# izhengfan/se2lam

Hardware: AMD Instinct MI355X
Metric: BA GN-iters/s (200 KF, 20k pts) (higher is better)
Workload: dtype f64; 1 GPU; globalBA-window 200 KF / 20000 landmarks / 119817 EdgeSE2XYZ + 199 PreEdgeSE2, LM optimize(10) (config 4 formulation, SURVEY D3); parallelism=single GPU

## Files before the change

### se2lam_amd/csrc/ba.hip

```cpp
#include <algorithm>
#include <atomic>
#include <chrono>
#include <cmath>
#include <cstdlib>
#include <functional>
#include <limits>
#include <mutex>
#include <thread>
#include <memory>
#include <unordered_map>

#include "common.h"
#include "se3_math.h"
#include "ba_device.h"
#include "ba3_device.h"
#include "ba_window.h"

using namespace se2gpu;
using namespace se2gpu::badev;

namespace {



// ... 2 lines not shown
    for (int r = 0; r < 3; ++r) {
        const double h0 = hh[r * 3], h1 = hh[r * 3 + 1], h2 = hh[r * 3 + 2];
        w[r * 3 + 0] = h0 * a[0];
        w[r * 3 + 1] = h0 * a[1] + h1 * a[2];
        w[r * 3 + 2] = h0 * a[3] + h1 * a[4] + h2 * a[5];
    }
}
__device__ __forceinline__ void edge_record(const double* __restrict__ hh, const double* __restrict__ hp,
                                            const double* __restrict__ bpe, const double a[6], const double zeta[3],
                                            double w[9], double dg[12]) {
    edge_w(hh, a, w);
    dg[0] = hp[0] - (w[0] * w[0] + w[1] * w[1] + w[2] * w[2]);
    dg[1] = hp[1] - (w[0] * w[3] + w[1] * w[4] + w[2] * w[5]);
    dg[2] = hp[2] - (w[0] * w[6] + w[1] * w[7] + w[2] * w[8]);
    dg[3] = hp[3] - (w[3] * w[3] + w[4] * w[4] + w[5] * w[5]);
    dg[4] = hp[4] - (w[3] * w[6] + w[4] * w[7] + w[5] * w[8]);
    dg[5] = hp[5] - (w[6] * w[6] + w[7] * w[7] + w[8] * w[8]);
#pragma unroll
    for (int r = 0; r < 3; ++r) {
        dg[6 + r] = bpe[r];
        dg[9 + r] = w[r * 3] * zeta[0] + w[r * 3 + 1] * zeta[1] + w[r * 3 + 2] * zeta[2];
    }
}
__device__ inline void write_edge_record(double* __restrict__ w_out, double* __restrict__ dg_out, const double* __restrict__ hh,
                                         const double* __restrict__ hp, const double* __restrict__ bpe,
                                         const double a[6], const double zeta[3]) {
    double w[9], dg[12];
    edge_record(hh, hp, bpe, a, zeta, w, dg);
#pragma unroll
    for (int i = 0; i < 9; ++i) w_out[i] = w[i];
#pragma unroll
    for (int i = 0; i < 12; ++i) dg_out[i] = dg[i];
}

__device__ __forceinline__ void wave_copy_out(double* __restrict__ dst, const double* stage, int n) {
    const int lane = threadIdx.x & 63;
    const int head = (int)((reinterpret_cast<uintptr_t>(dst) >> 3) & 1);
    if (lane == 0 && head) dst[0] = stage[0];
    const int nb = (n - head) >> 1;
    for (int i = lane; i < nb; i += 64) {
        const double2 v = make_double2(stage[head + 2 * i], stage[head + 2 * i + 1]);
        *reinterpret_cast<double2*>(dst + head + 2 * i) = v;
    }
    if (lane == 0 && ((n - head) & 1)) dst[n - 1] = stage[n - 1];
}

struct RecSet {
    double *W, *Dg, *Hll, *bl, *Ainv, *zeta;
};

__device__ __forceinline__ void lin_edge(const CamDev& cam, double px, double py, double pth, double lx, double ly, double lz,
                                         double u, double v, double w0, double w1, double w2, bool fr, double hll[6],
                                         double b[3], double hpl[9], double hpp[6], double bpe[3], double& r0) {
    double e0, e1, Jp[6], Jl[6];
    se2xyz<true>(cam, px, py, pth, lx, ly, lz, u, v, e0, e1, Jp, Jl);
// ... 42 lines not shown
        double* keep = lds + (threadIdx.x >> 6) * kWaveLds + (threadIdx.x & 63);
#pragma unroll
        for (int i = 0; i < 9; ++i) keep[i * 64] = hpl[i];
#pragma unroll
        for (int i = 0; i < 6; ++i) keep[(9 + i) * 64] = hpp[i];
#pragma unroll
        for (int i = 0; i < 3; ++i) keep[(15 + i) * 64] = bpe[i];
    } else {
        if (FUSED) {
#pragma unroll
            for (int i = 0; i < 9; ++i) W[(size_t)e * 9 + i] = hpl[i];
        }
#pragma unroll
        for (int i = 0; i < 6; ++i) Hpp_e[(size_t)e * 6 + i] = hpp[i];
#pragma unroll
        for (int i = 0; i < 3; ++i) bp_e[(size_t)e * 3 + i] = bpe[i];
    }
}

template <bool FUSED>
__device__ __forceinline__ void lin_landmark(int l, int sub, int beg, int end, int L, double hll[6], double b[3], double lambda,
                                             double* lds, double* W, double* Hpp_e, double* bp_e,
                                             double* __restrict__ Hll, double* __restrict__ bl, double* __restrict__ Ainv,
                                             double* __restrict__ zeta, double* __restrict__ Dg) {
#pragma unroll
    for (int i = 0; i < 6; ++i) hll[i] = group_sum(hll[i]);
#pragma unroll
    for (int i = 0; i < 3; ++i) b[i] = group_sum(b[i]);
    if (l < L && sub == 0) {
#pragma unroll
        for (int i = 0; i < 6; ++i) Hll[(size_t)l * 6 + i] = hll[i];
#pragma unroll
        for (int i = 0; i < 3; ++i) bl[(size_t)l * 3 + i] = b[i];
    }
    if (!FUSED) return;
    int e1 = l < L ? end : 0;
#pragma unroll
    for (int o = 32; o; o >>= 1) e1 = max(e1, __shfl_xor(e1, o));
    const int E0 = __builtin_amdgcn_readfirstlane(l < L ? beg : 0), E1 = __builtin_amdgcn_readfirstlane(e1);
    const int ne = E1 - E0;
    const bool staged = ne > 0 && ne <= kStageEdges;
    double* stage = lds + (threadIdx.x >> 6) * kWaveLds;
    const double* keep = stage + (threadIdx.x & 63);
    const bool has = l < L && beg + sub < end;
    double a[6] = {0, 0, 0, 0, 0, 0}, zt[3] = {0, 0, 0};
    if (l < L) {
        chol_inv3(hll, lambda, a);
        zt[0] = a[0] * b[0];
        zt[1] = a[1] * b[0] + a[2] * b[1];
        zt[2] = a[3] * b[0] + a[4] * b[1] + a[5] * b[2];
        if (sub == 0) {
#pragma unroll
            for (int i = 0; i < 6; ++i) Ainv[(size_t)l * 6 + i] = a[i];
#pragma unroll
            for (int i = 0; i < 3; ++i) zeta[(size_t)l * 3 + i] = zt[i];
        }
    }
    double w1[9], dg1[12];
    if (has) {
        double k_hpl[9], k_hpp[6], k_bp[3];
#pragma unroll
        for (int i = 0; i < 9; ++i) k_hpl[i] = keep[i * 64];
#pragma unroll
        for (int i = 0; i < 6; ++i) k_hpp[i] = keep[(9 + i) * 64];
#pragma unroll
        for (int i = 0; i < 3; ++i) k_bp[i] = keep[(15 + i) * 64];
        edge_record(k_hpl, k_hpp, k_bp, a, zt, w1, dg1);
    }
    const int lend = l < L ? end : 0;
    if (!staged) {
        if (has) {
#pragma unroll
            for (int i = 0; i < 9; ++i) W[(size_t)(beg + sub) * 9 + i] = w1[i];
#pragma unroll
            for (int i = 0; i < 12; ++i) Dg[(size_t)(beg + sub) * 12 + i] = dg1[i];
        }
        for (int e = beg + sub + kGroup; e < lend; e += kGroup) {
            double hh[9], hp[6], bpe[3];
#pragma unroll
            for (int i = 0; i < 9; ++i) hh[i] = W[(size_t)e * 9 + i];
#pragma unroll
            for (int i = 0; i < 6; ++i) hp[i] = Hpp_e[(size_t)e * 6 + i];
#pragma unroll
            for (int i = 0; i < 3; ++i) bpe[i] = bp_e[(size_t)e * 3 + i];
            write_edge_record(W + (size_t)e * 9, Dg + (size_t)e * 12, hh, hp, bpe, a, zt);
        }
        return;
    }
    __builtin_amdgcn_wave_barrier();
    if (has) {
#pragma unroll
        for (int i = 0; i < 12; ++i) stage[(beg + sub - E0) * 12 + i] = dg1[i];
    }
    for (int e = beg + sub + kGroup; e < lend; e += kGroup) {
        double hh[9], hp[6], bpe[3], w[9], dg[12];
#pragma unroll
        for (int i = 0; i < 9; ++i) hh[i] = W[(size_t)e * 9 + i];
#pragma unroll
        for (int i = 0; i < 6; ++i) hp[i] = Hpp_e[(size_t)e * 6 + i];
#pragma unroll
        for (int i = 0; i < 3; ++i) bpe[i] = bp_e[(size_t)e * 3 + i];
        edge_record(hh, hp, bpe, a, zt, w, dg);
#pragma unroll
        for (int i = 0; i < 12; ++i) stage[(e - E0) * 12 + i] = dg[i];
    }
    __builtin_amdgcn_wave_barrier();
    wave_copy_out(Dg + (size_t)E0 * 12, stage, ne * 12);
    __builtin_amdgcn_wave_barrier();
    if (has) {
#pragma unroll
        for (int i = 0; i < 9; ++i) stage[(beg + sub - E0) * 9 + i] = w1[i];
    }
    for (int e = beg + sub + kGroup; e < lend; e += kGroup) {
        double hh[9], w[9];
#pragma unroll
        for (int i = 0; i < 9; ++i) hh[i] = W[(size_t)e * 9 + i];
        edge_w(hh, a, w);
#pragma unroll
        for (int i = 0; i < 9; ++i) stage[(e - E0) * 9 + i] = w[i];
    }
    __builtin_amdgcn_wave_barrier();
    wave_copy_out(W + (size_t)E0 * 9, stage, ne * 9);
}

struct LinArgs {
    CamDev cam;
    int L;
    const int *lm_ptr, *e_kf;
    const double *e_uv, *e_info, *poses;
    const uint8_t* fixed;
    const double* lms;
    double *W, *Hpp_e, *bp_e, *Hll, *bl;
    double lambda;
    double *Ainv, *zeta, *Dg;
    const BaCtl* ctl;
    const double *poses_b, *lms_b;
    RecSet alt;
};
template <bool FUSED>
__device__ __forceinline__ void d_linearize(const unsigned bx, const LinArgs& a) {
    const double *poses = a.poses, *lms = a.lms;
    RecSet rec{a.W, a.Dg, a.Hll, a.bl, a.Ainv, a.zeta};
    double lambda = a.lambda;
    if constexpr (FUSED) asm volatile("" : "+s"(lambda));
    if (a.ctl) {
        if (a.ctl->done | a.ctl->rec_valid) return;
        if (a.ctl->sel) { poses = a.poses_b; lms = a.lms_b; }
        if (a.ctl->rec_sel) rec = a.alt;
        lambda = a.ctl->lambda;
    }
    const int gid = bx * kBlock + threadIdx.x;
    const int l = gid / kGroup, sub = gid % kGroup;
    double hll[6] = {0, 0, 0, 0, 0, 0}, b[3] = {0, 0, 0};
    __shared__ double keep[(kBlock / 64) * kWaveLds];
    int beg = 0, end = 0;
    if (l < a.L) {
        const double lx = lms[3 * l], ly = lms[3 * l + 1], lz = lms[3 * l + 2];
        beg = a.lm_ptr[l];
        end = a.lm_ptr[l + 1];
        for (int e = beg + sub; e < end; e += kGroup) {
            const int kf = a.e_kf[e];
            double hpl[9], hpp[6], bpe[3], r0;
            lin_edge(a.cam, poses[3 * kf], poses[3 * kf + 1], poses[3 * kf + 2], lx, ly, lz, a.e_uv[2 * e], a.e_uv[2 * e + 1],
                     a.e_info[3 * e], a.e_info[3 * e + 1], a.e_info[3 * e + 2], !a.fixed[kf], hll, b, hpl, hpp, bpe, r0);
            lin_park<FUSED>(e == beg + sub, e, hpl, hpp, bpe, keep, rec.W, a.Hpp_e, a.bp_e);
        }
    }
    lin_landmark<FUSED>(l, sub, beg, end, a.L, hll, b, lambda, keep, rec.W, a.Hpp_e, a.bp_e, rec.Hll, rec.bl, rec.Ainv, rec.zeta,
                        rec.Dg);
}
template <bool FUSED>
__global__ __launch_bounds__(kBlock) void k_linearize(LinArgs a) {
    d_linearize<FUSED>(blockIdx.x, a);
}


struct OdoArgs {
    int O;
    const int *o_i, *o_j;
    const double *o_meas, *o_info, *poses;
    const uint8_t* fixed;
    double *Oii, *Ojj, *Oij, *obi, *obj;
    const BaCtl* ctl;
    const double* poses_b;
};
__device__ __forceinline__ void d_odometry(const unsigned bx, const OdoArgs& a) {
    const double* poses = a.poses;
    if (a.ctl && a.ctl->sel) poses = a.poses_b;
    const int k = bx * blockDim.x + threadIdx.x;
    if (k >= a.O) return;
    const int i = a.o_i[k], j = a.o_j[k];
    double e[3], A[9], B[9];
// ... 192 lines not shown
    const int i = o_i[k], j = o_j[k];
    pre_se2(poses + 3 * i, poses + 3 * j, o_meas + 3 * k, e, A, B);
    const double* W = o_info + 9 * k;
    for (int r = 0; r < 3; ++r) {
        omr[r] = -(W[r * 3] * e[0] + W[r * 3 + 1] * e[1] + W[r * 3 + 2] * e[2]);
        for (int c = 0; c < 3; ++c) {
            WA[r * 3 + c] = W[r * 3] * A[c] + W[r * 3 + 1] * A[3 + c] + W[r * 3 + 2] * A[6 + c];
            WB[r * 3 + c] = W[r * 3] * B[c] + W[r * 3 + 1] * B[3 + c] + W[r * 3 + 2] * B[6 + c];
        }
    }
}

constexpr int kGrpPerWG = 28;
constexpr int kChunk = 16;

struct Reduce2Args {
    int P, ld, nwg_off;
    double lambda;
    int root;
    const int4* grp;
    const int *blk_a, *blk_b, *pair_i, *pair_j, *blk_odo;
    const double *W, *Dg;
    const uint8_t* fixed;
    const int *pose_ptr, *pose_edges, *podo_ptr, *podo_item, *o_i, *o_j;
    const double *o_meas, *o_info, *poses;
    double *S, *bp;
    const BaCtl* ctl;
    const double* poses_b;
    unsigned* epoch;
    const int* pose_off;
    int nsys;
    const double *W_alt, *Dg_alt;
};
__device__ __forceinline__ void d_reduce2(const unsigned bx, const Reduce2Args& ra) {
    const double *W = ra.W, *Dg = ra.Dg, *poses = ra.poses;
    if (ra.ctl && ra.ctl->rec_sel) { W = ra.W_alt; Dg = ra.Dg_alt; }
    double lambda = ra.lambda;
    const int n = ra.pose_off ? ra.nsys : 3 * ra.P;
    __shared__ double part[kGrpPerWG][9];
    __shared__ double dpart[kBlock / 64][12];
    const int ndiag = (ra.P + 1 + 7) & ~7;
    if ((int)bx >= ndiag) {
        const int bid = (int)bx - ndiag;
        const int nwg_pad = (ra.nwg_off + 7) & ~7;
        const int wg = (bid & 7) * (nwg_pad >> 3) + (bid >> 3);
        if (wg >= ra.nwg_off) return;
        const int lane = threadIdx.x & 63, gw = lane / 9, en = lane - 9 * gw;
// ... 94 lines not shown
    double acc[12] = {0, 0, 0, 0, 0, 0, 0, 0, 0, 0, 0, 0};
    const bool fa = ra.fixed[p];
    __shared__ double odoc[8][12];
    const int no = fa ? 0 : ra.podo_ptr[p + 1] - ra.podo_ptr[p];
    if ((int)threadIdx.x >= kBlock - 8 && (int)threadIdx.x - (kBlock - 8) < min(no, 8)) {
        const int t = ra.podo_ptr[p] + (int)threadIdx.x - (kBlock - 8);
        const int k = ra.podo_item[t] >> 1, isj = ra.podo_item[t] & 1;
        double e[3], A[9], B[9], WA[9], WB[9], omr[3];
        odo_terms(poses, ra.fixed, ra.o_i, ra.o_j, ra.o_meas, ra.o_info, k, e, A, B, WA, WB, omr);
        double J[9], WJ[9];
#pragma unroll
        for (int t9 = 0; t9 < 9; ++t9) { J[t9] = isj ? B[t9] : A[t9]; WJ[t9] = isj ? WB[t9] : WA[t9]; }
        double* o = odoc[threadIdx.x - (kBlock - 8)];
#pragma unroll
        for (int r = 0; r < 3; ++r) {
#pragma unroll
            for (int c = 0; c < 3; ++c) o[r * 3 + c] = J[r] * WJ[c] + J[3 + r] * WJ[3 + c] + J[6 + r] * WJ[6 + c];
            o[9 + r] = J[r] * omr[0] + J[3 + r] * omr[1] + J[6 + r] * omr[2];
        }
    }
    if (!fa) {
        const int e0 = ra.pose_ptr[p], ne = ra.pose_ptr[p + 1] - e0;
        for (int base = 0; base < ne; base += 4 * kBlock) {
            int ee[4];
            double wgt[4];
#pragma unroll
            for (int u = 0; u < 4; ++u) {
                const int t = base + u * kBlock + (int)threadIdx.x;
                wgt[u] = t < ne ? 1.0 : 0.0;
                ee[u] = ra.pose_edges[e0 + min(t, ne - 1)];
            }
#pragma unroll
            for (int u = 0; u < 4; ++u) {
                if (base + u * kBlock >= ne) break;
                const double2* rec = reinterpret_cast<const double2*>(Dg + (size_t)ee[u] * 12);
                const double w = wgt[u];
#pragma unroll
                for (int i = 0; i < 6; ++i) {
                    const double2 v = rec[i];
                    acc[2 * i] += w * v.x;
                    acc[2 * i + 1] += w * v.y;
                }
            }
        }
    }
#pragma unroll
    for (int i = 0; i < 12; ++i) acc[i] = wave_sum(acc[i]);
    if (lane == 0) {
#pragma unroll
        for (int i = 0; i < 12; ++i) dpart[wv][i] = acc[i];
    }
    __syncthreads();
    if (threadIdx.x < 12) {
        const int i = threadIdx.x;
        const int sym[9] = {0, 1, 2, 1, 3, 4, 2, 4, 5};
        const int src = i < 9 ? sym[i] : i - 3;
        double v = dpart[0][src] + dpart[1][src] + dpart[2][src] + dpart[3][src];
        for (int t = 0; t < min(no, 8); ++t) v += odoc[t][i];
        for (int t = ra.podo_ptr[p] + 8; t < ra.podo_ptr[p] + no; ++t) {
// ... 645 lines not shown
    TrialEnd te;
};
__device__ void finish_trial(const FinArgs& fin, const double* part, double lambda, double* fsp);

struct SpecArgs {
    RecSet set[2];
    double *Hpp_e, *bp_e;
};

struct UpdArgs {
    CamDev cam;
    int L;
    double lambda;
    const int *lm_ptr, *e_kf;
    const double *e_uv, *e_info, *poses;
    const uint8_t* fixed;
    const double *lms, *xp, *zeta, *W, *bl;
    double *lms_trial, *part;
    const BaCtl* ctl;
    const double* poses_b;
    FinArgs fin;
    const double* Ainv;
    SpecArgs sp;
};
template <bool LIN>
__device__ __forceinline__ void d_update(const unsigned bx, const UpdArgs& a) {
    __shared__ double lds[LIN ? (kBlock / 64) * kWaveLds : 3 * 1024];
    static_assert((kBlock / 64) * kWaveLds >= 3 * 1024, "the finisher's pose stage");
    if (a.fin.enabled && (int)bx == a.fin.nblk) {
        finish_trial(a.fin, a.part, a.lambda, lds);
        return;
    }
    const double *poses = a.poses, *lms = a.lms, *zeta = a.zeta, *W = a.W, *bl = a.bl, *Ainv = a.Ainv;
    double* lms_trial = a.lms_trial;
    double lambda = a.lambda;
    const int gid = bx * kBlock + threadIdx.x;
    const int l = gid / kGroup, sub = gid % kGroup;
    int beg = 0, end = 0;
    if (l < a.L) {
        beg = a.lm_ptr[l];
        end = a.lm_ptr[l + 1];
    }
    if (a.ctl) {
        if (a.ctl->done) return;
        if (a.ctl->sel) {
            const double* t = lms; lms = lms_trial; lms_trial = const_cast<double*>(t);
            poses = a.poses_b;
        }
        lambda = a.ctl->lambda;
    }
    const bool step = a.xp != nullptr;
    bool spec = false;
    double lambda_spec = 0;
    RecSet wr{};
    if (LIN && a.ctl && step) {
        spec = a.ctl->it + 1 < a.ctl->iters;
        lambda_spec = lm_lambda_spec(lambda, a.ctl->mode);
        const int rs = a.ctl->rec_sel;
        const RecSet rd = a.sp.set[rs];
        wr = a.sp.set[rs ^ 1];
        W = rd.W; zeta = rd.zeta; bl = rd.bl; Ainv = rd.Ainv;
    }
    double* keep = lds;
    double hll[6] = {0, 0, 0, 0, 0, 0}, bsum[3] = {0, 0, 0};
    __shared__ double sm[2][kBlock / 64];
    double chi = 0, scale = 0;
    double x[3] = {0, 0, 0};
    constexpr int KS = 2;
    int ekf[KS];
    bool ev[KS];
    double ey[KS][9], ep[KS][3], epose[KS][3], euv[KS][2], ew[KS][3];
    bool efix[KS];
#pragma unroll
    for (int k = 0; k < KS; ++k) {
        const int e = beg + sub + k * kGroup;
        ev[k] = e < end;
        const int ec = ev[k] ? e : max(end - 1, 0);
        const bool has = l < a.L && end > beg;
        ekf[k] = has ? a.e_kf[ec] : 0;
#pragma unroll
        for (int i = 0; i < 9; ++i) ey[k][i] = (has && step) ? W[(size_t)ec * 9 + i] : 0.0;
        euv[k][0] = has ? a.e_uv[2 * (size_t)ec] : 0.0;
        euv[k][1] = has ? a.e_uv[2 * (size_t)ec + 1] : 0.0;
#pragma unroll
        for (int i = 0; i < 3; ++i) ew[k][i] = has ? a.e_info[3 * (size_t)ec + i] : 0.0;
    }
#pragma unroll
    for (int k = 0; k < KS; ++k) {
        const int kf = ekf[k];
        epose[k][0] = poses[3 * kf]; epose[k][1] = poses[3 * kf + 1]; epose[k][2] = poses[3 * kf + 2];
        efix[k] = a.fixed[kf] != 0;
#pragma unroll
        for (int i = 0; i < 3; ++i) ep[k][i] = step ? a.xp[3 * kf + i] : 0.0;
    }
    double lw0[3] = {0, 0, 0}, zz[3] = {0, 0, 0}, blv[3] = {0, 0, 0}, av[6] = {0, 0, 0, 0, 0, 0};
    if (l < a.L) {
#pragma unroll
        for (int c = 0; c < 3; ++c) {
            lw0[c] = lms[(size_t)l * 3 + c];
            if (step) { zz[c] = zeta[(size_t)l * 3 + c]; blv[c] = bl[(size_t)l * 3 + c]; }
        }
        if (step) {
// ... 65 lines not shown
            edge_chi(e, poses[3 * kf], poses[3 * kf + 1], poses[3 * kf + 2], a.fixed[kf] != 0, dp, a.e_uv[2 * e], a.e_uv[2 * e + 1],
                     a.e_info[3 * e], a.e_info[3 * e + 1], a.e_info[3 * e + 2]);
        }
    }
    chi = wave_sum(chi);
    scale = wave_sum(scale);
    const int w = threadIdx.x / 64;
    if ((threadIdx.x & 63) == 0) { sm[0][w] = chi; sm[1][w] = scale; }
    __syncthreads();
    if (threadIdx.x == 0) {
        double c = 0, s = 0;
        for (int i = 0; i < kBlock / 64; ++i) { c += sm[0][i]; s += sm[1][i]; }
        if (a.fin.enabled) {
            store_agent(a.part + 2 * bx, d2_t{c, s});
            asm volatile("s_waitcnt vmcnt(0)" ::: "memory");
            __hip_atomic_fetch_add(a.fin.counter, 1u, __ATOMIC_RELAXED, __HIP_MEMORY_SCOPE_AGENT);
        } else {
            a.part[2 * bx] = c;
            a.part[2 * bx + 1] = s;
        }
    }
    if (LIN && spec)
        lin_landmark<true>(l, sub, beg, end, a.L, hll, bsum, lambda_spec, keep, wr.W, a.sp.Hpp_e, a.sp.bp_e, wr.Hll, wr.bl, wr.Ainv,
                           wr.zeta, wr.Dg);
}
template <bool LIN>
__global__ __launch_bounds__(kBlock) void k_update(UpdArgs a) {
    d_update<LIN>(blockIdx.x, a);
}

__global__ void k_ctl_clear_error(BaCtl* __restrict__ ctl) {
    ctl->error = 0;
    ctl->done = 0;
}

__device__ inline void post_ctl(const BaCtl* c, volatile double* mail, double seq, int tid, int nthr) {
    constexpr int kWords = (int)(sizeof(BaCtl) / 8);
    const double* src = reinterpret_cast<const double*>(c);
    for (int i = tid; i < kWords; i += nthr) mail[8 + i] = src[i];
}

__device__ inline void end_slot(BaCtl* ctl, volatile double* mail, bool post, int tid, int nthr, bool step) {
    if (!step) return;
    if (tid == 0) ctl->seq += 1.0;
    __syncthreads();
    if (post && mail) {
        __threadfence();
// ... 1011 lines not shown
    std::vector<int> pg_perm;
    DevBuf<int> slot_a, slot_ptr, pe_i, pe_j;
    DevBuf<double> pe_meas, pe_info, ph;
    int bulk_E = 0;
    const int32_t *bulk_kf = nullptr, *bulk_lm = nullptr;
    const double *bulk_uv = nullptr, *bulk_info = nullptr;
    bool lg_active = false;
    std::vector<float> lg_lc, lg_lw, lg_sigma2, lg_Rcw, lg_twb;
    float lg_fx = 0, lg_srot = 0, lg_sz = 0;
    DevBuf<float> d_lg_lc, d_lg_lw, d_lg_sigma2, d_lg_Rcw, d_lg_twb;
    std::vector<EdgeOdo> odo;
    bool initialized = false;
    unsigned long init_serial = 0;
    hipEvent_t join_event = nullptr;
    hipStream_t join_stream = nullptr;
    bool own_pending = false;
    int P = 0, L = 0, E = 0, O = 0, nblk = 0, nparts = 0;
    int ld = 0;
    bool host_solve = false;
    DevBuf<double> poses0, lms0, poses_a, poses_b, lms_a, lms_b;
    double *poses = nullptr, *poses_t = nullptr, *lms = nullptr, *lms_t = nullptr;
    DevBuf<uint8_t> fixed;
    DevBuf<int> lm_ptr, e_kf, e_lm, pose_ptr, pose_edges, podo_ptr, podo_item, o_i, o_j;
    DevBuf<int> blk_a, blk_b, blk_ptr, pair_i, pair_j, blk_odo;
    DevBuf<int4> grp;
    int nwg_off = 0, grp_cap_wg = 0;
    DevBuf<uint8_t> garena;
    DevBuf<int> plan_np, plan_base, plan_key0, plan_key1, plan_idx, plan_hist, plan_offs, plan_out, plan_tsum, plan_toff;
    DevBuf<int2> plan_st0, plan_st1;
    bool odo_fallback = false;
    bool odo_self_loop = false;
    DevBuf<double> e_uv, e_info, o_meas, o_info;
    DevBuf<double> Hpl, Hpp_e, bp_e, Hll, bl, Dinv, z, Y, Dg, Hpp, bp, Oii, Ojj, Oij, obi, obj;
    DevBuf<double> red_own, xp, part, scal, diag3, Rinv;
    DevBuf<double> rec_twin;
    bool run_spec = false;
    DevBuf<double> red_packed;
    DevBuf<int4> chol_tasks;
    DevBuf<int> chol_deps;
    DevBuf<int> chol_neager;
    DevBuf<int> pose_off;
    DevBuf<int> col_src;
    std::vector<int> h_pose_off;
    DevBuf<uint8_t> plan_nz;
    DevBuf<double> plan_nzd;
    PinBuf<uint8_t> h_plan_nz;
// ... 413 lines not shown
    if ((int)blockIdx.x < b1) {
        const int l = blockIdx.x * 256 + threadIdx.x;
        if (l >= L) return;
        int o = pair_base[l];
        const int beg = lm_ptr[l], end = lm_ptr[l + 1];
        for (int s = beg; s < end; ++s) {
            const int a = e_kf[s];
            if (fixed[a]) continue;
            for (int t = s + 1; t < end; ++t) {
                const int b = e_kf[t];
                if (fixed[b] || a == b) continue;
                const int q = a < b ? blk_index_of(P, a, b) : blk_index_of(P, b, a);
                key[o] = q;
                st[o] = a < b ? make_int2(s, t) : make_int2(t, s);
                if (nz) nz[q] = 1;
                ++o;
            }
        }
    } else {
        const int i = (blockIdx.x - b1) * 256 + threadIdx.x;
        if (i < cap && i >= pair_base[L]) key[i] = big;
    }
}
__global__ __launch_bounds__(256) void k_plan_bounds(const int* __restrict__ key, int n, int nq, int* __restrict__ out,
                                                      const int2* __restrict__ st, int* __restrict__ pi, int* __restrict__ pj,
                                                      int b1) {
    if ((int)blockIdx.x < b1) {
        const int q = blockIdx.x * 256 + threadIdx.x;
        if (q > nq) return;
        int lo = 0, hi = n;
        while (lo < hi) {
            const int mid = (lo + hi) >> 1;
            if (key[mid] < q) lo = mid + 1; else hi = mid;
        }
        out[q] = lo;
    } else {
        const int i = (blockIdx.x - b1) * 256 + threadIdx.x;
        if (i < n) { pi[i] = st[i].x; pj[i] = st[i].y; }
    }
}
inline dim3 grid1(size_t n, int block) { return dim3((unsigned)std::max<size_t>((n + block - 1) / block, 1)); }

__global__ void k_pattern_widen(int n, uint8_t* __restrict__ nz, double* __restrict__ d, int dir) {
    const int i = blockIdx.x * blockDim.x + threadIdx.x;
    if (i >= n) return;
    if (dir == 0) d[i] = nz[i] ? 1.0 : 0.0;
    else nz[i] = d[i] > 0.5 ? 1 : 0;
}
__global__ void k_solver_pads(double* __restrict__ S, int ld, int nsys, const int* __restrict__ col_src) {
    const int c = blockIdx.x * blockDim.x + threadIdx.x;
    if (c < nsys && col_src[c] < 0) S[(size_t)c * ld + c] = 1.0;
}

struct HostPlan {
    std::vector<int> lm_ptr, pose_ptr, pose_edges, blk_a, blk_b, blk_odo, pair_i, pair_j;
    std::vector<uint8_t> blk_nz;
    std::vector<int4> grp;
    int nwg_off = 0;
};
void ba_plan_host(int P, int L, int E, const int* e_kf, const int* e_lm, const uint8_t* fx, int O, const int* o_i,
                  const int* o_j, bool odo_ok, HostPlan& pl, int gpw = kGrpPerWG) {
    pl.lm_ptr.assign(L + 1, 0);
    for (int s = 0; s < E; ++s) pl.lm_ptr[e_lm[s] + 1]++;
    for (int l = 0; l < L; ++l) pl.lm_ptr[l + 1] += pl.lm_ptr[l];
    const std::vector<int>& lm_ptr = pl.lm_ptr;
    pl.pose_ptr.assign(P + 1, 0);
    pl.pose_edges.resize(E);
    for (int s = 0; s < E; ++s) pl.pose_ptr[e_kf[s] + 1]++;
    for (int p = 0; p < P; ++p) pl.pose_ptr[p + 1] += pl.pose_ptr[p];
    {
        std::vector<int> f(pl.pose_ptr.begin(), pl.pose_ptr.end() - 1);
        for (int s = 0; s < E; ++s) pl.pose_edges[f[e_kf[s]]++] = s;
    }
    const int nblk = P * (P + 1) / 2;
    std::vector<int> blk_ptr(nblk + 1, 0);
    pl.blk_a.resize(nblk);
    pl.blk_b.resize(nblk);
    for (int a = 0; a < P; ++a)
        for (int b = a; b < P; ++b) {
            pl.blk_a[blk_index_of(P, a, b)] = a;
            pl.blk_b[blk_index_of(P, a, b)] = b;
        }
    std::vector<int> pkey;
    std::vector<int2> pst;
    pkey.reserve(4 * (size_t)E);
    pst.reserve(4 * (size_t)E);
    for (int l = 0; l < L; ++l)
        for (int s = lm_ptr[l]; s < lm_ptr[l + 1]; ++s) {
            const int a = e_kf[s];
            if (fx[a]) continue;
            for (int t = s + 1; t < lm_ptr[l + 1]; ++t) {
                const int b = e_kf[t];
                if (fx[b] || a == b) continue;
                const int q = a < b ? blk_index_of(P, a, b) : blk_index_of(P, b, a);
                pkey.push_back(q);
                pst.push_back(a < b ? make_int2(s, t) : make_int2(t, s));
// ... 429 lines not shown
        stage(h->pe_j, pg_j.data(), pg_j.size());
        stage(h->pe_meas, pg_meas.data(), pg_meas.size());
        stage(h->pe_info, pg_info.data(), pg_info.size());
    }
    if (h->model) {
        stage(h->prior_has, h->h_prior_has.data(), h->h_prior_has.size());
        stage(h->prior_meas, h->h_prior_meas.data(), h->h_prior_meas.size());
        stage(h->prior_info, h->h_prior_info.data(), h->h_prior_info.size());
    }
    if (h->lg_active) {
        SE2_REQUIRE(sorted && h->lg_sigma2.size() == (size_t)E, SE2GPU_ERR_STATE,
                    "load_local_graph must not be mixed with add_edge calls");
        stage(h->d_lg_lc, h->lg_lc.data(), h->lg_lc.size());
        stage(h->d_lg_lw, h->lg_lw.data(), h->lg_lw.size());
        stage(h->d_lg_sigma2, h->lg_sigma2.data(), h->lg_sigma2.size());
        stage(h->d_lg_Rcw, h->lg_Rcw.data(), h->lg_Rcw.size());
        stage(h->d_lg_twb, h->lg_twb.data(), h->lg_twb.size());
    }
    if (!device_plan) {
        stage(h->grp, pl.grp.data(), pl.grp.size());
        stage(h->lm_ptr, pl.lm_ptr.data(), pl.lm_ptr.size());
        stage(h->pose_ptr, pl.pose_ptr.data(), pl.pose_ptr.size());
        stage(h->pose_edges, pl.pose_edges.data(), pl.pose_edges.size());
        stage(h->blk_a, pl.blk_a.data(), pl.blk_a.size());
        stage(h->blk_b, pl.blk_b.data(), pl.blk_b.size());
        stage(h->blk_odo, pl.blk_odo.data(), pl.blk_odo.size());
        stage(h->pair_i, pl.pair_i.data(), pl.pair_i.size());
        stage(h->pair_j, pl.pair_j.data(), pl.pair_j.size());
    }
    SE2_CHECK(h->poses_a.reserve((size_t)ps * P));
    SE2_CHECK(h->poses_b.reserve((size_t)ps * P));
    SE2_CHECK(h->lms_a.reserve(3 * (size_t)L + 1));
    SE2_CHECK(h->lms_b.reserve(3 * (size_t)L + 1));
    SE2_CHECK(h->Hpl.reserve((size_t)D * 3 * E + 1));
    if (h->model) SE2_CHECK(h->Y.reserve((size_t)D * 3 * E + 1));
    SE2_CHECK(h->Hpp_e.reserve((size_t)DS * E + 1));
    SE2_CHECK(h->bp_e.reserve((size_t)D * E + 1));
    SE2_CHECK(h->Dg.reserve((size_t)(DS + 2 * D) * E + 1));
    SE2_CHECK(h->Hll.reserve(6 * (size_t)L + 1));
    SE2_CHECK(h->bl.reserve(3 * (size_t)L + 1));
    SE2_CHECK(h->Dinv.reserve(6 * (size_t)L + 1));
    SE2_CHECK(h->z.reserve(3 * (size_t)L + 1));
    SE2_CHECK(h->Hpp.reserve((size_t)D * D * P));
    SE2_CHECK(h->bp.reserve((size_t)D * P));
    SE2_CHECK(h->diag3.reserve((size_t)D * P));
    SE2_CHECK(h->Oii.reserve((size_t)D * D * O + 1));
// ... 68 lines not shown
                done += nb;
                if (sg.off + done - sent >= kPiece) SE2_CHECK(flush_on(sg.off + done));
            }
        }
        return flush_on(std::min(hi, staged_bytes));
    };
    for (const Staged& sg : staged) sg.bind(h->garena.p + sg.off);
    SE2_CHECK(stage_range(0, big_off, st));
    lap("indices staged");
    bool pattern_early = false;
    if (h->lg_active && E)
        hipLaunchKernelGGL(k_edge_information, grid1(E, 256), dim3(256), 0, st, E, h->d_lg_lc.p, h->d_lg_lw.p, h->e_kf.p,
                           h->d_lg_sigma2.p, h->d_lg_Rcw.p, h->d_lg_twb.p, h->lg_fx, h->lg_srot, h->lg_sz, h->e_info.p, 1);
    if (device_plan) {
        const int Pb = std::max(1, (int)std::ceil(std::log2((double)std::max(P, 2))));
        const int Qb = std::max(2, (int)std::ceil(std::log2((double)nblk + 2.0)));
        const int qlo = (Qb + 1) / 2, qhi = Qb - qlo;
        SE2_REQUIRE(qlo <= 10 && Pb <= 10, SE2GPU_ERR_CAPACITY, "device plan: %d poses", P);
        const size_t NP = std::max<size_t>(npairs_max, 1);
        const int nblkE = (int)((E + kRadixItems - 1) / kRadixItems), nblkP = (int)((NP + kRadixItems - 1) / kRadixItems);
        SE2_CHECK(h->lm_ptr.reserve((size_t)L + 2));
        SE2_CHECK(h->pose_ptr.reserve((size_t)P + 2));
        SE2_CHECK(h->pose_edges.reserve((size_t)E + 1));
        SE2_CHECK(h->blk_a.reserve(nblk));
        SE2_CHECK(h->blk_b.reserve(nblk));
        SE2_CHECK(h->blk_odo.reserve(nblk));
        SE2_CHECK(h->blk_ptr.reserve((size_t)nblk + 2));
        SE2_CHECK(h->pair_i.reserve(NP));
        SE2_CHECK(h->pair_j.reserve(NP));
        SE2_CHECK(h->plan_np.reserve((size_t)L + 2));
        SE2_CHECK(h->plan_base.reserve((size_t)L + 2));
        SE2_CHECK(h->plan_key0.reserve(std::max<size_t>(NP, (size_t)E + 1)));
        SE2_CHECK(h->plan_key1.reserve(std::max<size_t>(NP, (size_t)E + 1)));
        SE2_CHECK(h->plan_st0.reserve(NP));
        SE2_CHECK(h->plan_st1.reserve(NP));
        SE2_CHECK(h->plan_idx.reserve((size_t)E + 1));
        const size_t nhist = (size_t)1024 * std::max(nblkE, nblkP) + 2;
        SE2_CHECK(h->plan_hist.reserve(nhist));
        SE2_CHECK(h->plan_offs.reserve(nhist));
        SE2_CHECK(h->plan_out.reserve(8));
        SE2_CHECK(h->plan_tsum.reserve(nhist / kScanTile + 4));
        SE2_CHECK(h->plan_toff.reserve(nhist / kScanTile + 4));
        const size_t G = npairs_max / kChunk + (size_t)P * (P - 1) / 2 + 1;
        const int cap_wg = (int)std::min<size_t>((size_t)P * (P - 1) / 2 + 1, 2 * G / gpw + 2) + 1;
        SE2_CHECK(h->grp.reserve((size_t)cap_wg * gpw));
        h->grp_cap_wg = cap_wg;
// ... 15 lines not shown
                               (int)cnt, shift, bins, nb, h->plan_offs.p, kout, vout);
            return SE2GPU_OK;
        };
        uint8_t* nzp = nullptr;
        if (nd_possible) {
            SE2_CHECK(h->plan_nz.reserve((size_t)nblk));
            SE2_CHECK(h->h_plan_nz.reserve((size_t)nblk));
            nzp = h->plan_nz.p;
        }
        {
            const int g1 = (int)grid1((size_t)L + 1, 256).x, g2 = (int)grid1(E, 256).x, g3 = (int)grid1((size_t)P * P, 256).x;
            const size_t ngrp = (size_t)cap_wg * gpw;
            const int g4 = (int)grid1(ngrp, 256).x;
            hipLaunchKernelGGL(k_plan_init, dim3(g1 + g2 + g3 + g4), dim3(256), 0, st, L, E, P, h->e_lm.p, h->e_kf.p, h->fixed.p,
                               h->lm_ptr.p, h->plan_np.p, h->plan_idx.p, h->blk_a.p, h->blk_b.p, h->blk_odo.p, ngrp, h->grp.p,
                               g1, g1 + g2, g1 + g2 + g3, nzp);
        }
        hipLaunchKernelGGL(k_scan_i32, dim3(1), dim3(1024), 0, st, h->plan_np.p, h->plan_base.p, L);
        if (O && (!h->odo_fallback || nzp))
            hipLaunchKernelGGL(k_plan_odo, grid1(O, 64), dim3(64), 0, st, P, O, h->o_i.p, h->o_j.p,
                               h->odo_fallback ? nullptr : h->blk_odo.p, nzp);
        if (E) SE2_CHECK(radix(h->e_kf.p, h->plan_key0.p, h->plan_idx.p, h->pose_edges.p, (size_t)E, 0, Pb));
        hipLaunchKernelGGL(k_lower_bounds, grid1((size_t)P + 1, 256), dim3(256), 0, st, h->plan_key0.p, E, P, h->pose_ptr.p);
        {
            const int g1 = (int)grid1(L, 256).x, g2 = (int)grid1(NP, 256).x;
            hipLaunchKernelGGL(k_plan_pairs2, dim3(g1 + g2), dim3(256), 0, st, L, P, h->lm_ptr.p, h->e_kf.p, h->fixed.p,
                               h->plan_base.p, h->plan_key0.p, h->plan_st0.p, (int)NP, nblk, g1, nzp);
        }
        if (nd_possible) {
            if (nd_sharded) {
                SE2_CHECK(h->plan_nzd.reserve((size_t)nblk));
                hipLaunchKernelGGL(k_pattern_widen, grid1((size_t)nblk, 256), dim3(256), 0, st, nblk, h->plan_nz.p, h->plan_nzd.p, 0);
                SE2_HIP(hipGetLastError());
                SE2_CHECK(ba_allreduce(h, h->plan_nzd.p, (size_t)nblk));
                hipLaunchKernelGGL(k_pattern_widen, grid1((size_t)nblk, 256), dim3(256), 0, st, nblk, h->plan_nz.p, h->plan_nzd.p, 1);
            }
            SE2_HIP(hipMemcpyAsync(h->h_plan_nz.p, h->plan_nz.p, (size_t)nblk, hipMemcpyDeviceToHost, st));
            SE2_HIP(hipEventRecord(h->ev_pat, st));
            pattern_early = true;
        }
        SE2_CHECK(radix(h->plan_key0.p, h->plan_key1.p, h->plan_st0.p, h->plan_st1.p, NP, 0, qlo));
        SE2_CHECK(radix(h->plan_key1.p, h->plan_key0.p, h->plan_st1.p, h->plan_st0.p, NP, qlo, std::max(qhi, 1)));
        {
            const int g1 = (int)grid1((size_t)nblk + 1, 256).x, g2 = (int)grid1(NP, 256).x;
            hipLaunchKernelGGL(k_plan_bounds, dim3(g1 + g2), dim3(256), 0, st, h->plan_key0.p, (int)NP, nblk, h->blk_ptr.p,
                               h->plan_st0.p, h->pair_i.p, h->pair_j.p, g1);
// ... 171 lines not shown
    for (unsigned i = t0; i < it.np; i += stride) it.dst_p[i] = it.src_p[i];
    for (unsigned i = t0; i < it.nl; i += stride) it.dst_l[i] = it.src_l[i];
}

struct Bufs {
    const BaCtl* c;
    double *pa, *pb, *la, *lb;
};
inline Bufs bufs(se2gpu_ba* h, bool ctl) {
    if (ctl) return Bufs{h->ctl.p, h->poses_a.p, h->poses_b.p, h->lms_a.p, h->lms_b.p};
    return Bufs{nullptr, h->poses, h->poses_t, h->lms, h->lms_t};
}

bool ba_env_speculate() {
    static const bool on = env_flag("SE2GPU_BA_SPECULATE", true);
    return on;
}
RecSet rec_own(const se2gpu_ba* h) { return RecSet{h->Hpl.p, h->Dg.p, h->Hll.p, h->bl.p, h->Dinv.p, h->z.p}; }
RecSet rec_twin(const se2gpu_ba* h) {
    if (!h->rec_twin.p || h->model) return RecSet{};
    const size_t E = (size_t)h->E, L = (size_t)h->L;
    double* p = h->rec_twin.p;
    RecSet r;
    r.W = p; p += 9 * E + 1;
    r.Dg = p; p += 12 * E + 1;
    r.Hll = p; p += 6 * L + 1;
    r.bl = p; p += 3 * L + 1;
    r.Ainv = p; p += 6 * L + 1;
    r.zeta = p;
    return r;
}
int ba_reserve_twin(se2gpu_ba* h) { return h->rec_twin.reserve(21 * (size_t)h->E + 18 * (size_t)h->L + 6); }

inline double* ba_scal(se2gpu_ba* h) { return h->red + (size_t)h->ld * h->ld; }
inline dim3 upd_grid(const se2gpu_ba* h) { return grid1((size_t)h->L * kGroup, kBlock); }
inline dim3 reduce2_grid(const se2gpu_ba* h) { return dim3(((h->P + 1 + 7) & ~7) + ((h->nwg_off + 7) & ~7)); }
LinArgs lin_args(se2gpu_ba* h, const Bufs& B, double lambda, const RecSet& alt) {
    return LinArgs{h->cam, h->L, h->lm_ptr.p, h->e_kf.p, h->e_uv.p, h->e_info.p, B.pa, h->fixed.p, B.la, h->Hpl.p, h->Hpp_e.p,
                   h->bp_e.p, h->Hll.p, h->bl.p, lambda, h->Dinv.p, h->z.p, h->Dg.p, B.c, B.pb, B.lb, alt};
}
OdoArgs odo_args(se2gpu_ba* h, const double* poses, bool ctl) {
    const Bufs B = bufs(h, ctl);
    return OdoArgs{h->O, h->o_i.p, h->o_j.p, h->o_meas.p, h->o_info.p, ctl ? B.pa : poses, h->fixed.p, h->Oii.p, h->Ojj.p, h->Oij.p,
                   h->obi.p, h->obj.p, B.c, ctl ? B.pb : nullptr};
}
PoseReduceArgs pose_reduce_args(se2gpu_ba* h) {
    return PoseReduceArgs{h->P, h->pose_ptr.p, h->pose_edges.p, h->Hpp_e.p, h->bp_e.p, h->podo_ptr.p, h->podo_item.p, h->Oii.p,
                          h->Ojj.p, h->obi.p, h->obj.p, h->Hpp.p, h->bp.p};
}
MaxdiagArgs maxdiag_args(se2gpu_ba* h, int dpp, int stride9, BaCtl* ctl) {
    return MaxdiagArgs{h->L, h->Hll.p, h->P, stride9 ? h->Hpp.p : h->diag3.p, h->fixed.p, h->scal.p, dpp, stride9, ctl};
}
Reduce2Args reduce2_args(se2gpu_ba* h, const Bufs& B, double lambda, const RecSet& alt) {
    return Reduce2Args{h->P, h->ld, h->nwg_off, lambda, h->root, h->grp.p, h->blk_a.p, h->blk_b.p, h->pair_i.p, h->pair_j.p,
                       h->blk_odo.p, h->Hpl.p, h->Dg.p, h->fixed.p, h->pose_ptr.p, h->pose_edges.p, h->podo_ptr.p, h->podo_item.p,
                       h->o_i.p, h->o_j.p, h->o_meas.p, h->o_info.p, B.pa, h->red, h->bp.p, B.c, B.pb, &h->ctl.p->epoch,
                       h->pose_off.p, h->nsys, alt.W, alt.Dg};
}
CholArgs chol_args(se2gpu_ba* h, const BaCtl* ctl, int skip, unsigned long long* head, bool verify) {
    const int n = h->nsys, ld = h->ld;
    const int nt = ld / kNB, nbc = (n + kNB - 1) / kNB;
    double* YU = h->Rinv.p + 2 * (size_t)nt * nbc * kSlabs * kSlabDoubles;
    unsigned* flagA = h->chol_flags.p;
    return CholArgs{h->red, h->Rinv.p, YU, ld, n, nbc, h->chol_tasks.p + skip, h->chol_deps.p, h->chol_neager.p + skip, h->col_src.p,
                    flagA, flagA + kSlabs * (size_t)nt * nbc, &h->ctl.p->epoch, ba_scal(h) + 2, h->chol_trace.p, ctl, h->xp.p,
                    verify ? h->chol_vfy.p : nullptr, head, h->chol_ntask - skip};
}
TrialEnd trial_end(se2gpu_ba* h, const Bufs& B, int step, int decide, int notify, double seq, bool lin = false, bool post = true) {
    return TrialEnd{ba_scal(h), post ? h->d_mail : nullptr, seq, B.c ? h->ctl.p : nullptr,
                    B.c ? (const volatile int*)h->d_stop : nullptr, step, decide, notify, lin ? 1 : 0};
}
FinArgs fin_args(se2gpu_ba* h, const Bufs& B, const double* xp, const TrialEnd& te) {
    return FinArgs{1, (int)upd_grid(h).x, h->P, h->O, h->root, h->fixed.p, xp, h->bp.p, B.pa, B.pb,
                   h->o_i.p, h->o_j.p, h->o_meas.p, h->o_info.p, h->fin_counter.p, te};
}
UpdArgs upd_args(se2gpu_ba* h, const Bufs& B, double lambda, const double* xp, const FinArgs& fin, bool lin = false) {
    return UpdArgs{h->cam, h->L, lambda, h->lm_ptr.p, h->e_kf.p, h->e_uv.p, h->e_info.p, B.pa, h->fixed.p, B.la, xp, h->z.p, h->Hpl.p,
                   h->bl.p, B.lb, h->part.p, B.c, B.pb, fin, h->Dinv.p,
                   lin ? SpecArgs{{rec_own(h), rec_twin(h)}, h->Hpp_e.p, h->bp_e.p} : SpecArgs{}};
}


int ba_linearize(se2gpu_ba* h, double fuse_lambda, bool ctl = false) {
    hipStream_t st = h->stream;
    const Bufs B = bufs(h, ctl);
    if (h->model == 2) {
        SE2_LAUNCH(h->prof, st, "k4_terms", k4_terms, grid1((size_t)h->P + h->O, 64), dim3(64), 0, h->P, h->O, B.pa, h->fixed.p,
                   h->prior_has.p, h->prior_meas.p, h->prior_info.p, h->ph.p, h->pb.p, h->slot_a.p, h->slot_ptr.p, h->pe_i.p,
                   h->pe_j.p, h->pe_meas.p, h->pe_info.p, h->Oii.p, h->Ojj.p, h->Oij.p, h->obi.p, h->obj.p, B.c, B.pb);
        SE2_HIP(hipGetLastError());
        return SE2GPU_OK;
    }
    if (h->model) {
        if (fuse_lambda >= 0.0)
            SE2_LAUNCH(h->prof, st, "k3_linearize", (k3_linearize<true>), grid1((size_t)h->L * kGroup, kBlock), dim3(kBlock), 0,
                       h->cam3, h->L, h->lm_ptr.p, h->e_kf.p, h->e_uv.p, h->e_info.p, B.pa, h->fixed.p, B.la, h->Hpl.p,
                       h->Hpp_e.p, h->bp_e.p, h->Hll.p, h->bl.p, fuse_lambda, h->Dinv.p, h->z.p, h->Y.p, h->Dg.p, B.c, B.pb, B.lb);
        else
            SE2_LAUNCH(h->prof, st, "k3_linearize", (k3_linearize<false>), grid1((size_t)h->L * kGroup, kBlock), dim3(kBlock), 0,
                       h->cam3, h->L, h->lm_ptr.p, h->e_kf.p, h->e_uv.p, h->e_info.p, B.pa, h->fixed.p, B.la, h->Hpl.p,
                       h->Hpp_e.p, h->bp_e.p, h->Hll.p, h->bl.p, 0.0, h->Dinv.p, h->z.p, h->Y.p, h->Dg.p, B.c, B.pb, B.lb);
        SE2_LAUNCH(h->prof, st, "k3_terms", k3_terms, grid1((size_t)h->P + h->O, 64), dim3(64), 0, h->P, h->O, B.pa, h->fixed.p,
// ... 1903 lines not shown
```

Baseline: 7222 iters/s.

## Store per-edge diagonal records in pose-sorted order via an edge slot map

Adds an e_slot permutation, built on host and device, that maps each landmark-ordered edge to its position in pose-sorted order. The linearize and update kernels now scatter the 12-double Dg records straight into that order with double2 stores. The pose reduction can then read Dg contiguously without the pose_edges gather, and the LDS staging and copy-out pass for Dg is dropped. The cost is scattered, uncoalesced writes on the producer side in exchange for coalesced reads in the reduction, plus an extra index load per edge and a realigned twin buffer layout.

```diff
diff --git a/se2lam_amd/csrc/ba.hip b/se2lam_amd/csrc/ba.hip
--- a/se2lam_amd/csrc/ba.hip
+++ b/se2lam_amd/csrc/ba.hip
@@ -48,15 +48,19 @@
         dg[9 + r] = w[r * 3] * zeta[0] + w[r * 3 + 1] * zeta[1] + w[r * 3 + 2] * zeta[2];
     }
 }
-__device__ inline void write_edge_record(double* __restrict__ w_out, double* __restrict__ dg_out, const double* __restrict__ hh,
-                                         const double* __restrict__ hp, const double* __restrict__ bpe,
-                                         const double a[6], const double zeta[3]) {
+__device__ __forceinline__ void store_diag_record(double* __restrict__ Dg, int slot, const double dg[12]) {
+    double2* d = reinterpret_cast<double2*>(Dg + (size_t)slot * 12);
+#pragma unroll
+    for (int i = 0; i < 6; ++i) d[i] = make_double2(dg[2 * i], dg[2 * i + 1]);
+}
+__device__ inline void write_edge_record(double* __restrict__ w_out, double* __restrict__ Dg, int slot,
+                                         const double* __restrict__ hh, const double* __restrict__ hp,
+                                         const double* __restrict__ bpe, const double a[6], const double zeta[3]) {
     double w[9], dg[12];
     edge_record(hh, hp, bpe, a, zeta, w, dg);
 #pragma unroll
     for (int i = 0; i < 9; ++i) w_out[i] = w[i];
-#pragma unroll
-    for (int i = 0; i < 12; ++i) dg_out[i] = dg[i];
+    store_diag_record(Dg, slot, dg);
 }
 
 __device__ __forceinline__ void wave_copy_out(double* __restrict__ dst, const double* stage, int n) {
@@ -145,7 +149,8 @@
 __device__ __forceinline__ void lin_landmark(int l, int sub, int beg, int end, int L, double hll[6], double b[3], double lambda,
                                              double* lds, double* W, double* Hpp_e, double* bp_e,
                                              double* __restrict__ Hll, double* __restrict__ bl, double* __restrict__ Ainv,
-                                             double* __restrict__ zeta, double* __restrict__ Dg) {
+                                             double* __restrict__ zeta, double* __restrict__ Dg,
+                                             const int* __restrict__ e_slot, int slot0) {
 #pragma unroll
     for (int i = 0; i < 6; ++i) hll[i] = group_sum(hll[i]);
 #pragma unroll
@@ -189,16 +194,16 @@
 #pragma unroll
         for (int i = 0; i < 3; ++i) k_bp[i] = keep[(15 + i) * 64];
         edge_record(k_hpl, k_hpp, k_bp, a, zt, w1, dg1);
+        store_diag_record(Dg, slot0, dg1);
     }
     const int lend = l < L ? end : 0;
     if (!staged) {
         if (has) {
 #pragma unroll
             for (int i = 0; i < 9; ++i) W[(size_t)(beg + sub) * 9 + i] = w1[i];
-#pragma unroll
-            for (int i = 0; i < 12; ++i) Dg[(size_t)(beg + sub) * 12 + i] = dg1[i];
         }
         for (int e = beg + sub + kGroup; e < lend; e += kGroup) {
+            const int slot = e_slot[e];
             double hh[9], hp[6], bpe[3];
 #pragma unroll
             for (int i = 0; i < 9; ++i) hh[i] = W[(size_t)e * 9 + i];
@@ -206,16 +211,17 @@
             for (int i = 0; i < 6; ++i) hp[i] = Hpp_e[(size_t)e * 6 + i];
 #pragma unroll
             for (int i = 0; i < 3; ++i) bpe[i] = bp_e[(size_t)e * 3 + i];
-            write_edge_record(W + (size_t)e * 9, Dg + (size_t)e * 12, hh, hp, bpe, a, zt);
+            write_edge_record(W + (size_t)e * 9, Dg, slot, hh, hp, bpe, a, zt);
         }
         return;
     }
     __builtin_amdgcn_wave_barrier();
     if (has) {
 #pragma unroll
-        for (int i = 0; i < 12; ++i) stage[(beg + sub - E0) * 12 + i] = dg1[i];
+        for (int i = 0; i < 9; ++i) stage[(beg + sub - E0) * 9 + i] = w1[i];
     }
     for (int e = beg + sub + kGroup; e < lend; e += kGroup) {
+        const int slot = e_slot[e];
         double hh[9], hp[6], bpe[3], w[9], dg[12];
 #pragma unroll
         for (int i = 0; i < 9; ++i) hh[i] = W[(size_t)e * 9 + i];
@@ -224,21 +230,7 @@
 #pragma unroll
         for (int i = 0; i < 3; ++i) bpe[i] = bp_e[(size_t)e * 3 + i];
         edge_record(hh, hp, bpe, a, zt, w, dg);
-#pragma unroll
-        for (int i = 0; i < 12; ++i) stage[(e - E0) * 12 + i] = dg[i];
-    }
-    __builtin_amdgcn_wave_barrier();
-    wave_copy_out(Dg + (size_t)E0 * 12, stage, ne * 12);
-    __builtin_amdgcn_wave_barrier();
-    if (has) {
-#pragma unroll
-        for (int i = 0; i < 9; ++i) stage[(beg + sub - E0) * 9 + i] = w1[i];
-    }
-    for (int e = beg + sub + kGroup; e < lend; e += kGroup) {
-        double hh[9], w[9];
-#pragma unroll
-        for (int i = 0; i < 9; ++i) hh[i] = W[(size_t)e * 9 + i];
-        edge_w(hh, a, w);
+        store_diag_record(Dg, slot, dg);
 #pragma unroll
         for (int i = 0; i < 9; ++i) stage[(e - E0) * 9 + i] = w[i];
     }
@@ -259,6 +251,7 @@
     const BaCtl* ctl;
     const double *poses_b, *lms_b;
     RecSet alt;
+    const int* e_slot;
 };
 template <bool FUSED>
 __device__ __forceinline__ void d_linearize(const unsigned bx, const LinArgs& a) {
@@ -276,13 +269,14 @@
     const int l = gid / kGroup, sub = gid % kGroup;
     double hll[6] = {0, 0, 0, 0, 0, 0}, b[3] = {0, 0, 0};
     __shared__ double keep[(kBlock / 64) * kWaveLds];
-    int beg = 0, end = 0;
+    int beg = 0, end = 0, slot0 = 0;
     if (l < a.L) {
         const double lx = lms[3 * l], ly = lms[3 * l + 1], lz = lms[3 * l + 2];
         beg = a.lm_ptr[l];
         end = a.lm_ptr[l + 1];
         for (int e = beg + sub; e < end; e += kGroup) {
             const int kf = a.e_kf[e];
+            if (FUSED && e == beg + sub) slot0 = a.e_slot[e];
             double hpl[9], hpp[6], bpe[3], r0;
             lin_edge(a.cam, poses[3 * kf], poses[3 * kf + 1], poses[3 * kf + 2], lx, ly, lz, a.e_uv[2 * e], a.e_uv[2 * e + 1],
                      a.e_info[3 * e], a.e_info[3 * e + 1], a.e_info[3 * e + 2], !a.fixed[kf], hll, b, hpl, hpp, bpe, r0);
@@ -290,7 +284,7 @@
         }
     }
     lin_landmark<FUSED>(l, sub, beg, end, a.L, hll, b, lambda, keep, rec.W, a.Hpp_e, a.bp_e, rec.Hll, rec.bl, rec.Ainv, rec.zeta,
-                        rec.Dg);
+                        rec.Dg, a.e_slot, slot0);
 }
 template <bool FUSED>
 __global__ __launch_bounds__(kBlock) void k_linearize(LinArgs a) {
@@ -529,7 +523,7 @@
     const int *blk_a, *blk_b, *pair_i, *pair_j, *blk_odo;
     const double *W, *Dg;
     const uint8_t* fixed;
-    const int *pose_ptr, *pose_edges, *podo_ptr, *podo_item, *o_i, *o_j;
+    const int *pose_ptr, *podo_ptr, *podo_item, *o_i, *o_j;
     const double *o_meas, *o_info, *poses;
     double *S, *bp;
     const BaCtl* ctl;
@@ -670,19 +664,12 @@
     if (!fa) {
         const int e0 = ra.pose_ptr[p], ne = ra.pose_ptr[p + 1] - e0;
         for (int base = 0; base < ne; base += 4 * kBlock) {
-            int ee[4];
-            double wgt[4];
-#pragma unroll
-            for (int u = 0; u < 4; ++u) {
-                const int t = base + u * kBlock + (int)threadIdx.x;
-                wgt[u] = t < ne ? 1.0 : 0.0;
-                ee[u] = ra.pose_edges[e0 + min(t, ne - 1)];
-            }
 #pragma unroll
             for (int u = 0; u < 4; ++u) {
                 if (base + u * kBlock >= ne) break;
-                const double2* rec = reinterpret_cast<const double2*>(Dg + (size_t)ee[u] * 12);
-                const double w = wgt[u];
+                const int t = base + u * kBlock + (int)threadIdx.x;
+                const double2* rec = reinterpret_cast<const double2*>(Dg + (size_t)(e0 + min(t, ne - 1)) * 12);
+                const double w = t < ne ? 1.0 : 0.0;
 #pragma unroll
                 for (int i = 0; i < 6; ++i) {
                     const double2 v = rec[i];
@@ -1374,6 +1361,7 @@
     FinArgs fin;
     const double* Ainv;
     SpecArgs sp;
+    const int* e_slot;
 };
 template <bool LIN>
 __device__ __forceinline__ void d_update(const unsigned bx, const UpdArgs& a) {
@@ -1419,7 +1407,7 @@
     double chi = 0, scale = 0;
     double x[3] = {0, 0, 0};
     constexpr int KS = 2;
-    int ekf[KS];
+    int ekf[KS], slot0 = 0;
     bool ev[KS];
     double ey[KS][9], ep[KS][3], epose[KS][3], euv[KS][2], ew[KS][3];
     bool efix[KS];
@@ -1430,6 +1418,7 @@
         const int ec = ev[k] ? e : max(end - 1, 0);
         const bool has = l < a.L && end > beg;
         ekf[k] = has ? a.e_kf[ec] : 0;
+        if (LIN && k == 0) slot0 = (spec && has) ? a.e_slot[ec] : 0;
 #pragma unroll
         for (int i = 0; i < 9; ++i) ey[k][i] = (has && step) ? W[(size_t)ec * 9 + i] : 0.0;
         euv[k][0] = has ? a.e_uv[2 * (size_t)ec] : 0.0;
@@ -1541,7 +1530,7 @@
     }
     if (LIN && spec)
         lin_landmark<true>(l, sub, beg, end, a.L, hll, bsum, lambda_spec, keep, wr.W, a.sp.Hpp_e, a.sp.bp_e, wr.Hll, wr.bl, wr.Ainv,
-                           wr.zeta, wr.Dg);
+                           wr.zeta, wr.Dg, a.e_slot, slot0);
 }
 template <bool LIN>
 __global__ __launch_bounds__(kBlock) void k_update(UpdArgs a) {
@@ -2599,6 +2588,7 @@
     double *poses = nullptr, *poses_t = nullptr, *lms = nullptr, *lms_t = nullptr;
     DevBuf<uint8_t> fixed;
     DevBuf<int> lm_ptr, e_kf, e_lm, pose_ptr, pose_edges, podo_ptr, podo_item, o_i, o_j;
+    DevBuf<int> e_slot;
     DevBuf<int> blk_a, blk_b, blk_ptr, pair_i, pair_j, blk_odo;
     DevBuf<int4> grp;
     int nwg_off = 0, grp_cap_wg = 0;
@@ -3058,6 +3048,10 @@
         if (i < cap && i >= pair_base[L]) key[i] = big;
     }
 }
+__global__ void k_edge_slots(const int* __restrict__ pose_edges, int E, int* __restrict__ e_slot) {
+    const int t = blockIdx.x * blockDim.x + threadIdx.x;
+    if (t < E) e_slot[pose_edges[t]] = t;
+}
 __global__ __launch_bounds__(256) void k_plan_bounds(const int* __restrict__ key, int n, int nq, int* __restrict__ out,
                                                       const int2* __restrict__ st, int* __restrict__ pi, int* __restrict__ pj,
                                                       int b1) {
@@ -3089,7 +3083,7 @@
 }
 
 struct HostPlan {
-    std::vector<int> lm_ptr, pose_ptr, pose_edges, blk_a, blk_b, blk_odo, pair_i, pair_j;
+    std::vector<int> lm_ptr, pose_ptr, pose_edges, e_slot, blk_a, blk_b, blk_odo, pair_i, pair_j;
     std::vector<uint8_t> blk_nz;
     std::vector<int4> grp;
     int nwg_off = 0;
@@ -3108,6 +3102,8 @@
         std::vector<int> f(pl.pose_ptr.begin(), pl.pose_ptr.end() - 1);
         for (int s = 0; s < E; ++s) pl.pose_edges[f[e_kf[s]]++] = s;
     }
+    pl.e_slot.resize(E);
+    for (int t = 0; t < E; ++t) pl.e_slot[pl.pose_edges[t]] = t;
     const int nblk = P * (P + 1) / 2;
     std::vector<int> blk_ptr(nblk + 1, 0);
     pl.blk_a.resize(nblk);
@@ -3583,6 +3579,7 @@
         stage(h->lm_ptr, pl.lm_ptr.data(), pl.lm_ptr.size());
         stage(h->pose_ptr, pl.pose_ptr.data(), pl.pose_ptr.size());
         stage(h->pose_edges, pl.pose_edges.data(), pl.pose_edges.size());
+        stage(h->e_slot, pl.e_slot.data(), pl.e_slot.size());
         stage(h->blk_a, pl.blk_a.data(), pl.blk_a.size());
         stage(h->blk_b, pl.blk_b.data(), pl.blk_b.size());
         stage(h->blk_odo, pl.blk_odo.data(), pl.blk_odo.size());
@@ -3697,6 +3694,7 @@
         SE2_CHECK(h->lm_ptr.reserve((size_t)L + 2));
         SE2_CHECK(h->pose_ptr.reserve((size_t)P + 2));
         SE2_CHECK(h->pose_edges.reserve((size_t)E + 1));
+        SE2_CHECK(h->e_slot.reserve((size_t)E + 1));
         SE2_CHECK(h->blk_a.reserve(nblk));
         SE2_CHECK(h->blk_b.reserve(nblk));
         SE2_CHECK(h->blk_odo.reserve(nblk));
@@ -3758,6 +3756,7 @@
                                h->odo_fallback ? nullptr : h->blk_odo.p, nzp);
         if (E) SE2_CHECK(radix(h->e_kf.p, h->plan_key0.p, h->plan_idx.p, h->pose_edges.p, (size_t)E, 0, Pb));
         hipLaunchKernelGGL(k_lower_bounds, grid1((size_t)P + 1, 256), dim3(256), 0, st, h->plan_key0.p, E, P, h->pose_ptr.p);
+        if (E) hipLaunchKernelGGL(k_edge_slots, grid1(E, 256), dim3(256), 0, st, h->pose_edges.p, E, h->e_slot.p);
         {
             const int g1 = (int)grid1(L, 256).x, g2 = (int)grid1(NP, 256).x;
             hipLaunchKernelGGL(k_plan_pairs2, dim3(g1 + g2), dim3(256), 0, st, L, P, h->lm_ptr.p, h->e_kf.p, h->fixed.p,
@@ -3975,22 +3974,22 @@
     const size_t E = (size_t)h->E, L = (size_t)h->L;
     double* p = h->rec_twin.p;
     RecSet r;
+    r.Dg = p; p += 12 * E + 2;
     r.W = p; p += 9 * E + 1;
-    r.Dg = p; p += 12 * E + 1;
     r.Hll = p; p += 6 * L + 1;
     r.bl = p; p += 3 * L + 1;
     r.Ainv = p; p += 6 * L + 1;
     r.zeta = p;
     return r;
 }
-int ba_reserve_twin(se2gpu_ba* h) { return h->rec_twin.reserve(21 * (size_t)h->E + 18 * (size_t)h->L + 6); }
+int ba_reserve_twin(se2gpu_ba* h) { return h->rec_twin.reserve(21 * (size_t)h->E + 18 * (size_t)h->L + 8); }
 
 inline double* ba_scal(se2gpu_ba* h) { return h->red + (size_t)h->ld * h->ld; }
 inline dim3 upd_grid(const se2gpu_ba* h) { return grid1((size_t)h->L * kGroup, kBlock); }
 inline dim3 reduce2_grid(const se2gpu_ba* h) { return dim3(((h->P + 1 + 7) & ~7) + ((h->nwg_off + 7) & ~7)); }
 LinArgs lin_args(se2gpu_ba* h, const Bufs& B, double lambda, const RecSet& alt) {
     return LinArgs{h->cam, h->L, h->lm_ptr.p, h->e_kf.p, h->e_uv.p, h->e_info.p, B.pa, h->fixed.p, B.la, h->Hpl.p, h->Hpp_e.p,
-                   h->bp_e.p, h->Hll.p, h->bl.p, lambda, h->Dinv.p, h->z.p, h->Dg.p, B.c, B.pb, B.lb, alt};
+                   h->bp_e.p, h->Hll.p, h->bl.p, lambda, h->Dinv.p, h->z.p, h->Dg.p, B.c, B.pb, B.lb, alt, h->e_slot.p};
 }
 OdoArgs odo_args(se2gpu_ba* h, const double* poses, bool ctl) {
     const Bufs B = bufs(h, ctl);
@@ -4006,7 +4005,7 @@
 }
 Reduce2Args reduce2_args(se2gpu_ba* h, const Bufs& B, double lambda, const RecSet& alt) {
     return Reduce2Args{h->P, h->ld, h->nwg_off, lambda, h->root, h->grp.p, h->blk_a.p, h->blk_b.p, h->pair_i.p, h->pair_j.p,
-                       h->blk_odo.p, h->Hpl.p, h->Dg.p, h->fixed.p, h->pose_ptr.p, h->pose_edges.p, h->podo_ptr.p, h->podo_item.p,
+                       h->blk_odo.p, h->Hpl.p, h->Dg.p, h->fixed.p, h->pose_ptr.p, h->podo_ptr.p, h->podo_item.p,
                        h->o_i.p, h->o_j.p, h->o_meas.p, h->o_info.p, B.pa, h->red, h->bp.p, B.c, B.pb, &h->ctl.p->epoch,
                        h->pose_off.p, h->nsys, alt.W, alt.Dg};
 }
@@ -4030,7 +4029,7 @@
 UpdArgs upd_args(se2gpu_ba* h, const Bufs& B, double lambda, const double* xp, const FinArgs& fin, bool lin = false) {
     return UpdArgs{h->cam, h->L, lambda, h->lm_ptr.p, h->e_kf.p, h->e_uv.p, h->e_info.p, B.pa, h->fixed.p, B.la, xp, h->z.p, h->Hpl.p,
                    h->bl.p, B.lb, h->part.p, B.c, B.pb, fin, h->Dinv.p,
-                   lin ? SpecArgs{{rec_own(h), rec_twin(h)}, h->Hpp_e.p, h->bp_e.p} : SpecArgs{}};
+                   lin ? SpecArgs{{rec_own(h), rec_twin(h)}, h->Hpp_e.p, h->bp_e.p} : SpecArgs{}, h->e_slot.p};
 }
 
 
```

Result: no change. 7282 iters/s (median of 6 runs) (+0.8%).
